# stm233/image-compression-for-machine

Hardware: AMD Instinct MI355X
Metric: images/sec (256x256) cnn-hyperprior (WACNN) training step (higher is better)
Workload: dtype f32; 1 GPU; cnn (WACNN N=192 M=320) train step, lambda=0.0067 MSE, batch 16/GPU synthetic 256x256, Adam lr 1e-4 + aux Adam, clip 1.0; global_batch=16, parallelism=dp1

## Files before the change

image-compression-for-machine_amd/csrc/conv_common.h:

```cpp
#pragma once
#include <type_traits>
#include "icm_common.h"

namespace icm {

#define ICM_MAX_TAPS 32
#define ICM_MAX_GROUPS 12

struct ConvPtrs {
  const float* x;
  const float* wp;
  const float* bias;
  float* y;
  const float* res;
  const float* aux;
  const float* aux2;
  float* y2;
};

struct ConvDesc {
  ConvPtrs g[ICM_MAX_GROUPS];
  long long y_bs, res_bs, aux_bs, aux2_bs, y2_bs;
  PatchGeom pg;
  int Cout, OHf, OWf;
// ... 81 lines not shown
template <int... Kinds>
struct EpiKinds {
  static constexpr bool has(int epi) { return ((epi == Kinds) || ...); }
  template <class F>
  static __device__ __forceinline__ void dispatch(int epi, F&& f) {
    static_assert(((Kinds == ICM_EPI_NONE) || ...), "ICM_EPI_NONE is the fallback of every kernel");
    const bool hit = ((Kinds != ICM_EPI_NONE && epi == Kinds ? (f(std::integral_constant<int, Kinds>{}), true) : false) || ...);
    if (!hit) f(std::integral_constant<int, ICM_EPI_NONE>{});
  }
};
using EpiAll = EpiKinds<ICM_EPI_NONE, ICM_EPI_RES, ICM_EPI_RES_GELU, ICM_EPI_GDN, ICM_EPI_IGDN, ICM_EPI_MUL_DGELU,
                        ICM_EPI_AXPY2, ICM_EPI_LRP, ICM_EPI_RES_MUL_DGELU>;
using EpiKs8 = EpiKinds<ICM_EPI_NONE, ICM_EPI_RES, ICM_EPI_RES_GELU, ICM_EPI_MUL_DGELU, ICM_EPI_LRP, ICM_EPI_RES_MUL_DGELU>;
using EpiWino = EpiKinds<ICM_EPI_NONE, ICM_EPI_RES, ICM_EPI_RES_GELU, ICM_EPI_MUL_DGELU, ICM_EPI_RES_MUL_DGELU, ICM_EPI_LRP>;

template <int EPI, int half>
__device__ __forceinline__ void store_half_e(const ConvDesc& d, const ConvPtrs& P, const f32x16 acc, int cot, int h,
                                             int n, int oy, int ox, bool pvalid) {
  const int plane = d.OHf * d.OWf;
  constexpr bool kRes = epi_reads_res(EPI), kAux = epi_reads_aux(EPI), kAux2 = epi_reads_aux2(EPI);
  float* yb = P.y + n * d.y_bs;
  const float* resb = kRes ? P.res + n * d.res_bs : nullptr;
  const float* auxb = kAux ? P.aux + n * d.aux_bs : nullptr;
  const float* aux2b = kAux2 ? P.aux2 + n * d.aux2_bs : nullptr;
  float* y2b = P.y2 ? P.y2 + n * d.y2_bs : nullptr;
  const bool has_bias = P.bias != nullptr;
  {
    int off[8];
    bool ok[8];
    float bv[8], rv[8], av[8];
#pragma unroll
    for (int q = 0; q < 8; ++q) {
      const int r = half * 8 + q;
      const int co = cot * 32 + (r & 3) + 8 * (r >> 2) + 4 * h;
      ok[q] = pvalid && co < d.Cout;
      off[q] = d.ps2 ? (co >> 2) * plane + (oy * 2 + ((co >> 1) & 1)) * d.OWf + ox * 2 + (co & 1)
                     : co * plane + oy * d.OWf + ox;
      bv[q] = (has_bias && ok[q]) ? P.bias[co] : 0.0f;
      if constexpr (kRes) rv[q] = ok[q] ? resb[off[q]] : 0.0f;
      if constexpr (kAux) av[q] = ok[q] ? auxb[off[q]] : 0.0f;
      if constexpr (kAux2) rv[q] = ok[q] ? aux2b[off[q]] : 0.0f;
    }
    float v[8];
#pragma unroll
    for (int q = 0; q < 8; ++q) {
      float side;
      v[q] = epi_apply<EPI>(acc[half * 8 + q] + bv[q], (kRes || kAux2) ? rv[q] : 0.0f, kAux ? av[q] : 0.0f, side);
      if constexpr (epi_writes_side(EPI))
        if (y2b && ok[q]) y2b[off[q]] = side;
    }
    if (d.accum) {
      float old[8];
#pragma unroll
      for (int q = 0; q < 8; ++q) old[q] = ok[q] ? yb[off[q]] : 0.0f;
#pragma unroll
      for (int q = 0; q < 8; ++q) v[q] += old[q];
    }
    if constexpr (epi_may_gelu(EPI)) {
      if (y2b) {
#pragma unroll
        for (int q = 0; q < 8; ++q) epi_materialise(v[q], yb, y2b, off[q], ok[q]);
      }
    }
#pragma unroll
    for (int q = 0; q < 8; ++q)
      if (ok[q]) yb[off[q]] = v[q];
  }
}
template <int EPI>
__device__ __forceinline__ void store_tile_e(const ConvDesc& d, const ConvPtrs& P, const f32x16 acc, int cot, int h,
                                             int n, int oy, int ox, bool pvalid) {
  store_half_e<EPI, 0>(d, P, acc, cot, h, n, oy, ox, pvalid);
  store_half_e<EPI, 1>(d, P, acc, cot, h, n, oy, ox, pvalid);
}

struct EpiRegs {
  int n;
  int off[8];
  bool ok[8];
  float bv[8], rv[8], av[8], old[8];
};

// ... 87 lines not shown
    epi_finish<EPI>(d, P, a8, R[i & 1]);
    __builtin_amdgcn_sched_barrier(0);
  }
}

template <int TCO, int TPX, bool PIPE2 = false>
__device__ __forceinline__ void epilogue_dispatch(const ConvDesc& d, const ConvPtrs& P, const f32x16 (&acc)[TCO][TPX],
                                                  int cot0, int h, const int (&pn)[TPX], const int (&poy)[TPX],
                                                  const int (&pox)[TPX], const bool (&pv)[TPX]) {
  EpiAll::dispatch(d.epi, [&](auto kind) {
    constexpr int EPI = decltype(kind)::value;
    epilogue_tiles<EPI, TCO, TPX, EPI == ICM_EPI_AXPY2 && PIPE2>(d, P, acc, cot0, h, pn, poy, pox, pv);
  });
}

int launch_conv_ks8(const ConvDesc& d, int tco, long long nblk, int ngroups, size_t lds_bytes, hipStream_t stream);

bool wino_supported(const icm_conv_args& a);
int plan_conv_wino(const icm_conv_args& a, int ngroups, WinoPlan& p);
int run_conv_wino(const icm_conv_args* arr, int ngroups, hipStream_t stream);
long long wino_transform_floats(const icm_conv_args& a);
int run_wino_transform(const icm_conv_args* arr, int ngroups, hipStream_t stream);

int plan_conv1x1(const icm_conv_args& a, int ngroups, int force_mode, ConvPlan& p);
int launch_conv1x1(ConvDesc& d, const icm_conv_args& a, const ConvPlan& p, int ngroups, hipStream_t stream);

}
```

image-compression-for-machine_amd/csrc/conv_igemm.hip:

```cpp
#include <cstdlib>
#include <vector>
#include "conv_common.h"

namespace icm {

template <int WCO, int WPX, int TCO, int TPX, int KS = 1>
__global__ __launch_bounds__(512, (TCO * TPX <= 3) ? 4 : 2) void conv_igemm_kernel(const ConvDesc d) {
  extern __shared__ __attribute__((aligned(16))) float smem[];
  static_assert(WCO * WPX * KS == 4, "4 MFMA waves per workgroup");
  constexpr int BCO_T = WCO * TCO;
  constexpr int TS = (TCO * TPX == 1) ? 3 : ((TCO * TPX == 2) ? 2 : 1);
  const int tid = threadIdx.x, lane = tid & 63, wave = tid >> 6;
  const bool loader = wave >= 4;
  const ConvPtrs P = d.g[blockIdx.y];
  const PatchGeom& pg = d.pg;

  int bid = xcd_block_id();
  const int cb = bid % d.ncb;
  int pt = bid / d.ncb;
  const int tx_i = pt % d.tiles_x;
  pt /= d.tiles_x;
  const int ty_i = pt % d.tiles_y;
  const int tn_i = pt / d.tiles_y;
  const int ox0 = tx_i << d.lgTW, oy0 = ty_i << d.lgTH, n0 = tn_i << d.lgTI;
// ... 460 lines not shown
  static const long long ks8_min = env_ll("ICM_CONV_KS8_MINWG", 160);
  if (!(ks8_forced() || (ks8_on && !cfg_forced())) || S_in != 1 || s.ntaps <= 1 || a.pro_act != ICM_ACT_NONE ||
      !EpiKs8::has(a.epi) || a.x_seg_len != 0)
    return 0;
  const int tco = g_force_cfg == ICM_CONV_CFG_KS8_32X128 ? 1 : (g_force_cfg == ICM_CONV_CFG_KS8_64X64 ? 2 : (s.ncot >= 2 ? 2 : 1));
  g = make_geometry(tco == 2 ? 64 : 128, s.OHv, s.OWv, a.N, S_in, cls.ey, cls.ex, s.nchunks8, s.ntaps, 4);
  int ckm = std::max(1, std::min(s.nchunks8, 64 / s.ntaps));
  while (ckm > 1 && (size_t)2 * ckm * 8 * g.CS * sizeof(float) > 96 * 1024) --ckm;
  g.ckm = ckm;
  g.lds_bytes = std::max((size_t)2 * ckm * 8 * g.CS * sizeof(float), (size_t)8 * 4 * 16 * 64 * sizeof(float));
  const long long blocks = cdiv(s.ncot, tco) * tile_count(g) * ngroups;
  const bool fits = g.lds_bytes <= 160 * 1024 && fits_plane_map(g) && linear_patch(g);
  return (fits && (ks8_forced() || (blocks <= ks8_max && blocks >= ks8_min && tco == 2))) ? tco : 0;
}

static int plan_class(const icm_conv_args& a, int ngroups, const ConvClass& cls, int S_in, int out_s, bool x_aligned16,
                      ConvPlan& p) {
  p = ConvPlan{};
  const ClassShape s = class_shape(a, cls, out_s);
  if (s.OHv <= 0 || s.OWv <= 0) return ICM_OK;
  if (s.ntaps > ICM_MAX_TAPS) return ICM_ERR_UNSUPPORTED;
  if (s.ntaps == 1 && S_in == 1 && out_s == 1 && cls.iy0 == 0 && cls.ix0 == 0 && a.x_seg_len == 0 && !cfg_forced()) {
    const int rc = plan_conv1x1(a, ngroups, g_force_1x1, p);
    if (rc >= 0) return rc;
  }
  p.row = search_staged(a, ngroups, cls, s, S_in, p.g);
  if (p.row < 0) return ICM_ERR_UNSUPPORTED;
  p.block = 512;
  Geometry kg;
  if (const int tco = plan_ks8(a, ngroups, cls, s, S_in, kg)) {
    p.family = kFamKs8;
    p.row = tco;
    p.g = kg;
    p.dma = 1;
  } else {
    const Geometry& g = p.g;
// ... 35 lines not shown
  d.OHf = d.ps2 ? a.OH * 2 : a.OH;
  d.OWf = d.ps2 ? a.OW * 2 : a.OW;
  d.OHv = s.OHv; d.OWv = s.OWv;
  d.out_sy = d.out_sx = out_s;
  d.out_oy = cls.cy; d.out_ox = cls.cx;
  d.iy0 = cls.iy0; d.ix0 = cls.ix0;
  d.ntaps = s.ntaps;
  d.lgTW = bg.lgTW; d.lgTH = bg.lgTH; d.lgTI = bg.lgTI;
  d.tiles_x = bg.tiles_x; d.tiles_y = bg.tiles_y; d.tiles_n = bg.tiles_n;
  d.nchunks8 = s.nchunks8; d.ckm = bg.ckm;
  for (int t = 0; t < s.ntaps; ++t) {
    const Tap& tp = cls.taps[t];
    const int col = (S_in == 2) ? ((tp.dx & 1) * bg.PWh + (tp.dx >> 1)) : tp.dx;
    d.tapoff[t] = tp.dy * bg.PWrow + col;
  }
  if (p.family == kFamKs8) return launch_conv_ks8(d, p.row, p.nblk, ngroups, bg.lds_bytes, stream);
  const KernelCfg& c = kCfgs[p.row];
  if (bg.lds_bytes > 64 * 1024 && !ensure_max_lds(reinterpret_cast<const void*>(c.fn))) return ICM_ERR_LAUNCH;
  hipLaunchKernelGGL(c.fn, dim3((unsigned)p.nblk, ngroups, 1), dim3(p.block), bg.lds_bytes, stream, d);
  ICM_CHECK_LAUNCH();
  return ICM_OK;
}

static int validate(const icm_conv_args& a) {
  if (!a.x || !a.wp || !a.y) return ICM_ERR_ARG;
  if (a.N <= 0 || a.Cin <= 0 || a.Cout <= 0 || a.H <= 0 || a.W <= 0 || a.OH <= 0 || a.OW <= 0) return ICM_ERR_ARG;
  if (a.KH <= 0 || a.KW <= 0 || a.KH * a.KW > ICM_MAX_TAPS) return ICM_ERR_UNSUPPORTED;
  if (a.stride != 1 && a.stride != 2) return ICM_ERR_UNSUPPORTED;
  if (!a.transposed) {
    if (a.OH != (a.H + 2 * a.pad - a.KH) / a.stride + 1 || a.OW != (a.W + 2 * a.pad - a.KW) / a.stride + 1)
      return ICM_ERR_ARG;
// ... 14 lines not shown
    if (rc) return rc;
  }
  const icm_conv_args& a = arr[0];
  for (int i = 1; i < ngroups; ++i) {
    const icm_conv_args& b = arr[i];
    if (b.N != a.N || b.Cin != a.Cin || b.H != a.H || b.W != a.W || b.Cout != a.Cout || b.OH != a.OH || b.OW != a.OW ||
        b.KH != a.KH || b.KW != a.KW || b.stride != a.stride || b.pad != a.pad || b.transposed != a.transposed ||
        b.pro_act != a.pro_act || b.epi != a.epi || b.accum != a.accum || b.pixel_shuffle != a.pixel_shuffle ||
        b.x_bs != a.x_bs || b.y_bs != a.y_bs || b.x_seg_len != a.x_seg_len || b.x_seg_gap != a.x_seg_gap || b.algo != a.algo ||
        (b.res && b.res_bs != a.res_bs) || (b.aux && b.aux_bs != a.aux_bs) || (b.aux2 && b.aux2_bs != a.aux2_bs) ||
        (b.y2 && b.y2_bs != a.y2_bs) || (b.res != nullptr) != (a.res != nullptr) || (b.aux != nullptr) != (a.aux != nullptr) ||
        (b.aux2 != nullptr) != (a.aux2 != nullptr) || (b.y2 != nullptr) != (a.y2 != nullptr) ||
        (b.bias != nullptr) != (a.bias != nullptr) || (b.xv != nullptr) != (a.xv != nullptr))
      return ICM_ERR_ARG;
  }
  return (a.algo == ICM_ALGO_WINOGRAD || a.algo == ICM_ALGO_DIRECT) ? ICM_OK : ICM_ERR_ARG;
}

static long long class_packed_floats(int Cin, int ntaps, int ncot) { return (long long)cdiv(Cin, 8) * ntaps * ncot * 256; }

static bool x_aligned16(const icm_conv_args* arr, int ngroups) {
  bool ok = true;
  for (int gi = 0; gi < ngroups; ++gi) ok = ok && (reinterpret_cast<uintptr_t>(arr[gi].x) & 15) == 0;
  return ok;
}

static int conv_run_grouped(const icm_conv_args* arr, int ngroups, hipStream_t stream) {
  if (int rc = check_group(arr, ngroups)) return rc;
  const icm_conv_args& a = arr[0];
  if (a.algo == ICM_ALGO_WINOGRAD) return run_conv_wino(arr, ngroups, stream);
  const int S_in = a.transposed ? 1 : a.stride, out_s = a.transposed ? a.stride : 1;
// ... 38 lines not shown
}
int icm_convT2d_dgrad(const icm_conv_args* a, void* stream) {
  if (!a || a->transposed) return ICM_ERR_ARG;
  return icm_conv_run(a, stream);
}
int icm_conv2d_dgrad(const icm_conv_args* a, void* stream) {
  if (!a || !a->transposed) return ICM_ERR_ARG;
  return icm_conv_run(a, stream);
}
int icm_convT2d_fwd(const icm_conv_args* a, void* stream) {
  if (!a || !a->transposed) return ICM_ERR_ARG;
  return icm_conv_run(a, stream);
}

int icm_conv_winograd_ok(const icm_conv_args* a) { return (a && icm::wino_supported(*a)) ? 1 : 0; }
int64_t icm_wino_transform_floats(const icm_conv_args* a) {
  return (a && icm::wino_supported(*a) && a->N > 0 && a->Cin > 0) ? (int64_t)icm::wino_transform_floats(*a) : -1;
}
int icm_wino_transform(const icm_conv_args* arr, int ngroups, void* stream) {
  if (!arr || ngroups < 1 || ngroups > ICM_MAX_GROUPS) return ICM_ERR_ARG;
  for (int i = 1; i < ngroups; ++i)
    if (arr[i].N != arr[0].N || arr[i].Cin != arr[0].Cin || arr[i].H != arr[0].H || arr[i].W != arr[0].W ||
        arr[i].x_bs != arr[0].x_bs || arr[i].pro_act != arr[0].pro_act || arr[i].x_seg_len != arr[0].x_seg_len ||
        arr[i].x_seg_gap != arr[0].x_seg_gap)
      return ICM_ERR_ARG;
  return icm::run_wino_transform(arr, ngroups, (hipStream_t)stream);
}

void icm_debug_force_conv_cfg(int idx) { icm::g_force_cfg = idx < 0 ? ICM_CONV_CFG_AUTO : idx; }
int icm_debug_forced_conv_cfg(void) { return icm::g_force_cfg; }
// ... 98 lines not shown
```

image-compression-for-machine_amd/csrc/conv_ks8.hip:

```cpp
#include <cstdlib>
#include "conv_common.h"

namespace icm {

template <int EPI>
__device__ __forceinline__ void ks8_store(const ConvDesc& d, const ConvPtrs& P, const f32x16 v, int cot, int hf, int h, int n,
                                          int oy, int ox, bool pvalid) {
  if (hf == 0) store_half_e<EPI, 0>(d, P, v, cot, h, n, oy, ox, pvalid);
  else store_half_e<EPI, 1>(d, P, v, cot, h, n, oy, ox, pvalid);
}

template <int TCO, int TPX>
__global__ __launch_bounds__(512, 2) void conv_ks8_kernel(const ConvDesc d) {
  extern __shared__ __attribute__((aligned(16))) float smem[];
  static_assert(TCO * TPX == 4, "four output tiles per workgroup: one half tile per wave in the epilogue");
  const int tid = threadIdx.x, lane = tid & 63;
  const int wave = __builtin_amdgcn_readfirstlane(tid >> 6);
  const ConvPtrs P = d.g[blockIdx.y];
  const PatchGeom& pg = d.pg;
  int bid = xcd_block_id();
  const int cb = bid % d.ncb;
  int pt = bid / d.ncb;
  const int tx_i = pt % d.tiles_x;
  pt /= d.tiles_x;
  const int ty_i = pt % d.tiles_y;
  const int tn_i = pt / d.tiles_y;
  const int ox0 = tx_i << d.lgTW, oy0 = ty_i << d.lgTH, n0 = tn_i << d.lgTI;
  const int iyb = oy0 + d.iy0, ixb = ox0 + d.ix0;
  const int bufsz = d.ckm * 8 * pg.CS;
  const int nchunks = (d.nchunks8 + d.ckm - 1) / d.ckm;
  const long long HWb = (long long)pg.H * pg.W * 4;
  const float* zero = icm_zero_page + lane;
  const int nj = (pg.TIPH * pg.PW + 63) >> 6;

  PlaneMap pm;
  plane_map_init(pm, pg, n0, iyb, ixb, lane);
  const char* xb = reinterpret_cast<const char*>(P.x);
  auto stage = [&](int chunk) {
    const int c0 = chunk * d.ckm * 8;
    const int nch = min(d.ckm, d.nchunks8 - chunk * d.ckm) * 8;
    float* dst = smem + (chunk & 1) * bufsz;
    for (int cl = wave; cl < nch; cl += 8) {
      const int c = c0 + cl;
      const char* base = xb + (long long)c * HWb;
      float* slab = dst + cl * pg.CS;
#pragma unroll
      for (int j = 0; j < ICM_MAXJ; ++j) {
        if (j < nj && pm.loff[j] >= 0) {
          const float* pp = (c < pg.C && pm.goff[j] >= 0) ? reinterpret_cast<const float*>(base + pm.goff[j]) : zero;
          __builtin_amdgcn_global_load_lds(pp, slab + 64 * j, 4, 0, 0);
        }
      }
    }
  };

  const int h = lane >> 5, l31 = lane & 31;
  const int TWm = (1 << d.lgTW) - 1, THm = (1 << d.lgTH) - 1;
  int boff[TPX];
#pragma unroll
// ... 65 lines not shown
            acc[a][tp] = __builtin_amdgcn_mfma_f32_32x32x2f32(aq[u][a][j], bv[j][tp], acc[a][tp], 0, 0, 0);
        aq[u][a] = *reinterpret_cast<const f32x4*>(sp + wl[a]);
      }
    }
  }
  while (chunk + 1 < nchunks) cross();
  asm volatile("s_waitcnt vmcnt(0)" ::: "memory");
  __syncthreads();

  float* red = smem;
#pragma unroll
  for (int a = 0; a < TCO; ++a)
#pragma unroll
    for (int tp = 0; tp < TPX; ++tp)
#pragma unroll
      for (int r = 0; r < 16; ++r) red[((wave * 4 + a * TPX + tp) * 16 + r) * 64 + lane] = acc[a][tp][r];
  __syncthreads();
  const int t = wave >> 1, hf = wave & 1;
  f32x16 v;
#pragma unroll
  for (int r = 0; r < 16; ++r) v[r] = 0.0f;
#pragma unroll
  for (int q = 0; q < 8; ++q) {
    float s = 0.0f;
#pragma unroll
    for (int k = 0; k < 8; ++k) s += red[((k * 4 + t) * 16 + hf * 8 + q) * 64 + lane];
    if (hf == 0) v[q] = s; else v[8 + q] = s;
  }
  const int a_t = t / TPX, tp_t = t % TPX;
  const int cot = cot0 + a_t;
  const int p = tp_t * 32 + l31;
  const int tx = p & TWm, ty = (p >> d.lgTW) & THm, ti = p >> (d.lgTW + d.lgTH);
  const int n = n0 + ti, oyv = oy0 + ty, oxv = ox0 + tx;
  const bool pvalid = (n < pg.N) && (oyv < d.OHv) && (oxv < d.OWv) && cot < d.ncot;
  const int oy = oyv * d.out_sy + d.out_oy, ox = oxv * d.out_sx + d.out_ox;
  EpiKs8::dispatch(d.epi, [&](auto kind) { ks8_store<decltype(kind)::value>(d, P, v, cot, hf, h, n, oy, ox, pvalid); });
}

int launch_conv_ks8(const ConvDesc& d, int tco, long long nblk, int ngroups, size_t lds_bytes, hipStream_t stream) {
  void (*fn)(const ConvDesc) = tco == 2 ? conv_ks8_kernel<2, 2> : conv_ks8_kernel<1, 4>;
  if (lds_bytes > 64 * 1024 && !ensure_max_lds(reinterpret_cast<const void*>(fn))) return ICM_ERR_LAUNCH;
  hipLaunchKernelGGL(fn, dim3((unsigned)nblk, ngroups, 1), dim3(512), lds_bytes, stream, d);
  ICM_CHECK_LAUNCH();
  return ICM_OK;
}

}
```

image-compression-for-machine_amd/icm_amd/_lib.py:

```python
from __future__ import annotations

import ctypes as C
import os

import torch

_HERE = os.path.dirname(os.path.abspath(__file__))
LIB_PATH = os.environ.get("ICM_LIB", os.path.join(os.path.dirname(_HERE), "lib", "libicm_hip.so"))

ACT_NONE, ACT_GELU, ACT_SQUARE = 0, 1, 2
CONV_CFG_AUTO, CONV_CFG_KS8_64X64, CONV_CFG_KS8_32X128 = -1, 100, 101
TILE_EDGE_LEFT, TILE_EDGE_RIGHT, TILE_EDGE_TOP, TILE_EDGE_BOTTOM = 1, 2, 4, 8
EPI_NONE, EPI_RES, EPI_RES_GELU, EPI_GDN, EPI_IGDN, EPI_MUL_DGELU, EPI_AXPY2, EPI_LRP, EPI_RES_MUL_DGELU = range(9)

_f = C.POINTER(C.c_float)
i64, i32, f32, vp = C.c_int64, C.c_int, C.c_float, C.c_void_p


class ConvArgs(C.Structure):
    _fields_ = [
        ("x", vp), ("x_bs", i64), ("N", i32), ("Cin", i32), ("H", i32), ("W", i32),
        ("wp", vp), ("bias", vp),
        ("y", vp), ("y_bs", i64), ("Cout", i32), ("OH", i32), ("OW", i32),
        ("KH", i32), ("KW", i32), ("stride", i32), ("pad", i32),
        ("transposed", i32), ("pro_act", i32), ("epi", i32),
        ("res", vp), ("res_bs", i64), ("aux", vp), ("aux_bs", i64), ("aux2", vp), ("aux2_bs", i64),
# ... 26 lines not shown
    _fields_ = [("matrix", vp * 5), ("bias", vp * 5), ("factor", vp * 4), ("dmedian", vp)]


class IcmError(RuntimeError):
    pass


_lib = None

SYMBOLS = [
    "icm_strerror", "icm_version", "icm_conv_run", "icm_conv_run_grouped", "icm_conv2d_fwd", "icm_conv2d_dgrad",
    "icm_convT2d_fwd", "icm_convT2d_dgrad", "icm_packed_weight_floats", "icm_pack_weights", "icm_pack_weights_batch",
    "icm_wgrad_workspace_floats", "icm_wgrad_workspace_floats_grouped", "icm_conv_wgrad", "icm_conv_wgrad_grouped", "icm_channel_sum", "icm_nonneg_fwd", "icm_nonneg_bwd",
    "icm_gdn_bwd_pre", "icm_gelu_fwd", "icm_gate_fwd", "icm_gate_bwd", "icm_add_grad", "icm_ste_round_offset",
    "icm_lrp_bwd", "icm_pixel_unshuffle2", "icm_layernorm_fwd", "icm_layernorm_bwd", "icm_space_to_depth2",
    "icm_residual_scale", "icm_im2col", "icm_col2im", "icm_copy_strided", "icm_permute_flip", "icm_gather_vectors", "icm_conv_winograd_ok", "icm_wino_transform_floats", "icm_wino_transform", "icm_winattn_fwd", "icm_winattn_bwd",
    "icm_eb_likelihood_fwd", "icm_eb_likelihood_bwd", "icm_eb_aux_loss", "icm_gc_likelihood_ste_fwd",
    "icm_gc_likelihood_ste_bwd", "icm_rd_loss_fwd", "icm_rd_loss_bwd", "icm_grad_sqnorm", "icm_adam_step", "icm_adam_step_hyper", "icm_fill",
    "icm_winattn_bwd_workspace_floats", "icm_debug_force_conv_cfg", "icm_debug_forced_conv_cfg", "icm_debug_force_conv1x1",
    "icm_debug_force_wgrad_cfg", "icm_debug_wgrad_plan", "icm_debug_conv_plan",
    "icm_debug_force_winattn_valu", "icm_debug_winattn_route",
    "icm_zigzag_order", "icm_zigzag_splits", "icm_zigzag_reverse",
    "icm_pmf_to_quantized_cdf", "icm_rans_encode_with_indexes", "icm_rans_decode_with_indexes",
    "icm_rans_decoder_create", "icm_rans_decoder_decode", "icm_rans_decoder_destroy",
    "icm_rans_lanes_waves", "icm_rans_lanes_encode", "icm_rans_lanes_decoder_create",
    "icm_rans_lanes_decoder_decode_run", "icm_rans_lanes_decoder_finish", "icm_rans_lanes_decoder_destroy",
    "icm_rans_lanes_encode_gpu_workspace", "icm_rans_lanes_encode_gpu", "icm_rans_lanes_decoder_gpu_create",
    "icm_rans_lanes_decoder_gpu_decode_run", "icm_rans_lanes_decoder_gpu_finish", "icm_rans_lanes_decoder_gpu_destroy",
    "icm_debug_lanes_search",
    "icm_eb_table_bounds", "icm_eb_pmf_table", "icm_gc_table_centers", "icm_gc_pmf_table", "icm_gc_build_indexes",
    "icm_quantize", "icm_dequantize", "icm_clamp", "icm_pad2d",
# ... 11 lines not shown
    if _lib is None:
        if not os.path.exists(LIB_PATH):
            raise IcmError(
                f"{LIB_PATH} not found: build it with image-compression-for-machine_amd/build.sh "
                "(hipcc --offload-arch=gfx950). There is no CPU fallback.")
        L = C.CDLL(LIB_PATH)
        L.icm_strerror.restype = C.c_char_p
        L.icm_packed_weight_floats.restype = i64
        L.icm_wgrad_workspace_floats.restype = i64
        L.icm_wgrad_workspace_floats_grouped.restype = i64
        L.icm_packed_weight_floats.argtypes = [i32, i32, i32, i32]
        L.icm_pack_weights.argtypes = [vp, vp, i32, i32, i32, i32, i32, i32, i32, i32, i32, f32, f32, vp]
        L.icm_pack_weights_batch.argtypes = [C.POINTER(PackJob), i32, vp]
        L.icm_conv_run.argtypes = [C.POINTER(ConvArgs), vp]
        L.icm_conv_winograd_ok.argtypes = [C.POINTER(ConvArgs)]
        L.icm_wino_transform_floats.argtypes = [C.POINTER(ConvArgs)]
        L.icm_wino_transform_floats.restype = i64
        L.icm_wino_transform.argtypes = [C.POINTER(ConvArgs), i32, vp]
        L.icm_conv_run_grouped.argtypes = [C.POINTER(ConvArgs), i32, vp]
        for n in ("icm_conv2d_fwd", "icm_conv2d_dgrad", "icm_convT2d_fwd", "icm_convT2d_dgrad"):
            getattr(L, n).argtypes = [C.POINTER(ConvArgs), vp]
        L.icm_wgrad_workspace_floats.argtypes = [C.POINTER(WgradArgs)]
        L.icm_wgrad_workspace_floats_grouped.argtypes = [C.POINTER(WgradArgs), i32]
        L.icm_conv_wgrad.argtypes = [C.POINTER(WgradArgs), vp]
        L.icm_conv_wgrad_grouped.argtypes = [C.POINTER(WgradArgs), i32, vp]
        L.icm_channel_sum.argtypes = [vp, i64, i32, i32, i32, vp, i32, vp, i64, vp]
        L.icm_gather_vectors.argtypes = [C.POINTER(vp), i32, i32, vp, vp]
        L.icm_nonneg_fwd.argtypes = [vp, vp, i64, f32, f32, vp]
        L.icm_nonneg_bwd.argtypes = [vp, vp, vp, i64, f32, i32, vp]
        L.icm_gdn_bwd_pre.argtypes = [vp, vp, vp, vp, vp, i64, i32, vp]
# ... 138 lines not shown
```

image-compression-for-machine_amd/icm_amd/engine.py:

```python
from __future__ import annotations

import ctypes as C
import os as _os
from typing import Callable, Dict, List, Optional, Sequence, Tuple

import torch

from . import _lib as L
from ._lib import (ACT_GELU, ACT_NONE, ACT_SQUARE, EPI_AXPY2, EPI_GDN, EPI_IGDN, EPI_LRP, EPI_MUL_DGELU, EPI_NONE,
                   EPI_RES, EPI_RES_GELU, EPI_RES_MUL_DGELU, bs, check, ptr)
from .bitstream import step_of, step_table

PEDESTAL = 2.0 ** -36
_SKIP_WGRAD = _os.environ.get("ICM_DEBUG_SKIP_WGRAD", "0") == "1"
PAIR_GATE_BRANCHES = _os.environ.get("ICM_PAIR_GATE_BRANCHES", "1") == "1"


MAX_GROUP = 12


USE_WINO = _os.environ.get("ICM_WINO", "1") != "0"
_WINO_MIN_CIN = int(_os.environ.get("ICM_WINO_MIN_CIN", "96"))
_WINO_MIN_WORK = float(_os.environ.get("ICM_WINO_MIN_WORK", "2.0e8"))
_WINO_WG_BATCH = float(_os.environ.get("ICM_WINO_WG_BATCH", "4"))
USE_WINO_WGRAD = _os.environ.get("ICM_WINO_WGRAD", "1") != "0"
THIN_OUT = _os.environ.get("ICM_THIN_OUT", "1") != "0"
EVAL_INPLACE_ACT = _os.environ.get("ICM_EVAL_INPLACE_ACT", "1") != "0"
WINO_PRE = _os.environ.get("ICM_WINO_PRE", "1") != "0"
_WINO_WG_MAX_PIXELS = int(_os.environ.get("ICM_WINO_WG_MAX_PIXELS", "100000"))


_WINO_WG_MIN_C = int(_os.environ.get("ICM_WINO_WG_MIN_C", "64"))


def wino_ok(KH, KW, stride, pad, Cin, ps=0, conv_transposed=False, work: float = 1e30, min_c=None) -> bool:
    return (USE_WINO and KH == 3 and KW == 3 and stride == 1 and pad == 1 and not ps and not conv_transposed and
            Cin >= (_WINO_MIN_CIN if min_c is None else min_c) and work >= _WINO_MIN_WORK and
            L.lib().icm_debug_forced_conv_cfg() == L.CONV_CFG_AUTO)


_weight_gen = [0]


def bump_weight_generation():
    _weight_gen[0] += 1


PROFILE: Optional[list] = None


def _prof_begin(stream=None):
    if PROFILE is None:
        return None
# ... 278 lines not shown
        a.accum, a.pixel_shuffle, a.algo = accum, ps, algo
        if biases is not None:
            a.bias = ptr(biases[i])
        if ress is not None:
            a.res, a.res_bs = ptr(ress[i]), bs(ress[i])
        if auxs is not None:
            a.aux, a.aux_bs = ptr(auxs[i]), bs(auxs[i])
        if aux2s is not None:
            a.aux2, a.aux2_bs = ptr(aux2s[i]), bs(aux2s[i])
        if y2s is not None:
            a.y2, a.y2_bs = ptr(y2s[i]), bs(y2s[i])
        if seg is not None:
            a.x_seg_len, a.x_seg_gap = seg
    if n > 1 and len({(m.x_bs, m.y_bs, m.res_bs, m.aux_bs, m.aux2_bs, m.y2_bs) for m in arr}) > 1:
        raise ValueError("grouped conv: members must share strides")
    if algo and WINO_PRE:
        _wino_pretransform(tape, arr, xs)
    if single:
        check(L.lib().icm_conv_run(C.byref(arr[0]), tape.st), "conv_run")
    else:
        check(L.lib().icm_conv_run_grouped(arr, n, tape.st), "conv_run_grouped")
    if e0 is not None:
        N, _, H, W = xs[0].shape
        px = H * W if transposed else OH * OW
        _prof_end(e0, _conv_label(tag + ("/wino" if algo else ""), transposed, KH, stride, Cin, Cout, H, W, N, n),
                  2.0 * n * N * Cin * Cout * KH * KW * px)


def conv_launch_grouped(tape, xs, wps, biases, ys, **kw):
    _conv_launch(tape, False, xs, wps, biases, ys, **kw)


def conv_launch(tape, x, wp, bias, y, *, res=None, aux=None, aux2=None, y2=None, **kw):
    one = lambda t: None if t is None else (t,)
    _conv_launch(tape, True, (x,), (wp,), one(bias), (y,), ress=one(res), auxs=one(aux), aux2s=one(aux2), y2s=one(y2),
                 **kw)


def _wgrad_args(a, gs, gb, dw, geom, accum, dbias, accum_bias, dw_ld=0, algo=0):
    Ca, Cb, KH, KW, stride, pad, act_s, act_b, N, OH, OW, H, W, gs_bs, gb_bs = geom
# ... 875 lines not shown
```

include/icm_hip.h:

```cpp
#ifndef ICM_HIP_H
#define ICM_HIP_H
#include <stdint.h>

#ifdef __cplusplus
extern "C" {
#endif

#define ICM_OK 0
#define ICM_ERR_ARG 1
#define ICM_ERR_LAUNCH 2
#define ICM_ERR_UNSUPPORTED 3

#define ICM_ACT_NONE 0
#define ICM_ACT_GELU 1
#define ICM_ACT_SQUARE 2

#define ICM_EPI_NONE 0
#define ICM_EPI_RES 1
#define ICM_EPI_RES_GELU 2
#define ICM_EPI_GDN 3
#define ICM_EPI_IGDN 4
#define ICM_EPI_MUL_DGELU 5
#define ICM_EPI_AXPY2 6
#define ICM_EPI_LRP 7
// ... 11 lines not shown
  int transposed;
  int pro_act;
  int epi;
  const float* res; int64_t res_bs;
  const float* aux; int64_t aux_bs;
  const float* aux2; int64_t aux2_bs;
  float* y2; int64_t y2_bs;
  int accum;
  int pixel_shuffle;
  int x_seg_len, x_seg_gap;
  int algo;
  float* xv;
} icm_conv_args;
#define ICM_ALGO_DIRECT 0
#define ICM_ALGO_WINOGRAD 1
int icm_conv_winograd_ok(const icm_conv_args* a);
int64_t icm_wino_transform_floats(const icm_conv_args* a);
int icm_wino_transform(const icm_conv_args* arr, int ngroups, void* stream);

int icm_conv_run(const icm_conv_args* a, void* stream);
int icm_conv_run_grouped(const icm_conv_args* a, int ngroups, void* stream);
int icm_conv2d_fwd(const icm_conv_args* a, void* stream);
int icm_conv2d_dgrad(const icm_conv_args* a, void* stream);
int icm_convT2d_fwd(const icm_conv_args* a, void* stream);
int icm_convT2d_dgrad(const icm_conv_args* a, void* stream);

int64_t icm_packed_weight_floats(int Cout, int Cin, int KH, int KW);
int icm_pack_weights(const float* w, float* wp, int Cout, int Cin, int KH, int KW, int src_out_major,
                     int transposed, int stride, int pad, int nonneg, float bound, float pedestal,
                     void* stream);

// ... 199 lines not shown
#define ICM_TILE_EDGE_LEFT 1
#define ICM_TILE_EDGE_RIGHT 2
#define ICM_TILE_EDGE_TOP 4
#define ICM_TILE_EDGE_BOTTOM 8
int icm_image_tile_blend(const float* src, int PH, int PW, int top, int left, int h, int w,
                         float* canvas, int H, int W, int y0, int x0,
                         const float* ramp, int m, int edges, void* stream);

typedef struct { int64_t offset; int32_t H, W, y0, x0; } icm_crop_desc;
int icm_image_batch_u8_to_f32(const uint8_t* arena, const icm_crop_desc* desc, int B, float* dst ,
                              int CH, int CW, void* stream);

#define ICM_CONV_CFG_AUTO (-1)
#define ICM_CONV_CFG_KS8_64X64 100
#define ICM_CONV_CFG_KS8_32X128 101
void icm_debug_force_conv_cfg(int idx);
int icm_debug_forced_conv_cfg(void);
void icm_debug_force_conv1x1(int mode);
int icm_debug_conv_plan(const icm_conv_args* a, int ngroups, int cls, int64_t out[16]);
void icm_debug_force_wgrad_cfg(int variant, int xcd_order);
int icm_debug_wgrad_plan(const icm_wgrad_args* a, int n, int32_t out[8]);
void icm_debug_force_winattn_valu(int on);
int icm_debug_winattn_route(int N, int C, int H, int W, int heads, int ws, int shift, int backward);

#ifdef __cplusplus
}
#endif
#endif
```

Measured before the change: 386.7 images/s.

## Add split-K conv path with smaller tile shapes for low-occupancy layers

Adds an ICM_ALGO_KSPLIT path that routes small-tile-count convolutions to the 8-wave split-K kernel. The kernel is generalized to 1, 2 or 4 output tiles per workgroup, and a planner picks the shape that best fills one round of workgroups. The Python engine enables the path by default for layers within tile, step and Cout thresholds. The aim is better GPU occupancy on small-spatial layers whose tile count underfills the device, at the cost of an LDS reduction across waves and heuristic thresholds that may misroute some layers.

```diff
diff --git a/image-compression-for-machine_amd/csrc/conv_common.h b/image-compression-for-machine_amd/csrc/conv_common.h
--- a/image-compression-for-machine_amd/csrc/conv_common.h
+++ b/image-compression-for-machine_amd/csrc/conv_common.h
@@ -119,9 +119,9 @@
 using EpiKs8 = EpiKinds<ICM_EPI_NONE, ICM_EPI_RES, ICM_EPI_RES_GELU, ICM_EPI_MUL_DGELU, ICM_EPI_LRP, ICM_EPI_RES_MUL_DGELU>;
 using EpiWino = EpiKinds<ICM_EPI_NONE, ICM_EPI_RES, ICM_EPI_RES_GELU, ICM_EPI_MUL_DGELU, ICM_EPI_RES_MUL_DGELU, ICM_EPI_LRP>;
 
-template <int EPI, int half>
-__device__ __forceinline__ void store_half_e(const ConvDesc& d, const ConvPtrs& P, const f32x16 acc, int cot, int h,
-                                             int n, int oy, int ox, bool pvalid) {
+template <int EPI, int NR>
+__device__ __forceinline__ void store_rows_e(const ConvDesc& d, const ConvPtrs& P, const float (&a8)[NR], int r0, int cot,
+                                             int h, int n, int oy, int ox, bool pvalid) {
   const int plane = d.OHf * d.OWf;
   constexpr bool kRes = epi_reads_res(EPI), kAux = epi_reads_aux(EPI), kAux2 = epi_reads_aux2(EPI);
   float* yb = P.y + n * d.y_bs;
@@ -131,12 +131,12 @@
   float* y2b = P.y2 ? P.y2 + n * d.y2_bs : nullptr;
   const bool has_bias = P.bias != nullptr;
   {
-    int off[8];
-    bool ok[8];
-    float bv[8], rv[8], av[8];
-#pragma unroll
-    for (int q = 0; q < 8; ++q) {
-      const int r = half * 8 + q;
+    int off[NR];
+    bool ok[NR];
+    float bv[NR], rv[NR], av[NR];
+#pragma unroll
+    for (int q = 0; q < NR; ++q) {
+      const int r = r0 + q;
       const int co = cot * 32 + (r & 3) + 8 * (r >> 2) + 4 * h;
       ok[q] = pvalid && co < d.Cout;
       off[q] = d.ps2 ? (co >> 2) * plane + (oy * 2 + ((co >> 1) & 1)) * d.OWf + ox * 2 + (co & 1)
@@ -146,31 +146,39 @@
       if constexpr (kAux) av[q] = ok[q] ? auxb[off[q]] : 0.0f;
       if constexpr (kAux2) rv[q] = ok[q] ? aux2b[off[q]] : 0.0f;
     }
-    float v[8];
-#pragma unroll
-    for (int q = 0; q < 8; ++q) {
+    float v[NR];
+#pragma unroll
+    for (int q = 0; q < NR; ++q) {
       float side;
-      v[q] = epi_apply<EPI>(acc[half * 8 + q] + bv[q], (kRes || kAux2) ? rv[q] : 0.0f, kAux ? av[q] : 0.0f, side);
+      v[q] = epi_apply<EPI>(a8[q] + bv[q], (kRes || kAux2) ? rv[q] : 0.0f, kAux ? av[q] : 0.0f, side);
       if constexpr (epi_writes_side(EPI))
         if (y2b && ok[q]) y2b[off[q]] = side;
     }
     if (d.accum) {
-      float old[8];
-#pragma unroll
-      for (int q = 0; q < 8; ++q) old[q] = ok[q] ? yb[off[q]] : 0.0f;
-#pragma unroll
-      for (int q = 0; q < 8; ++q) v[q] += old[q];
+      float old[NR];
+#pragma unroll
+      for (int q = 0; q < NR; ++q) old[q] = ok[q] ? yb[off[q]] : 0.0f;
+#pragma unroll
+      for (int q = 0; q < NR; ++q) v[q] += old[q];
     }
     if constexpr (epi_may_gelu(EPI)) {
       if (y2b) {
 #pragma unroll
-        for (int q = 0; q < 8; ++q) epi_materialise(v[q], yb, y2b, off[q], ok[q]);
+        for (int q = 0; q < NR; ++q) epi_materialise(v[q], yb, y2b, off[q], ok[q]);
       }
     }
 #pragma unroll
-    for (int q = 0; q < 8; ++q)
+    for (int q = 0; q < NR; ++q)
       if (ok[q]) yb[off[q]] = v[q];
   }
+}
+template <int EPI, int half>
+__device__ __forceinline__ void store_half_e(const ConvDesc& d, const ConvPtrs& P, const f32x16 acc, int cot, int h,
+                                             int n, int oy, int ox, bool pvalid) {
+  float a8[8];
+#pragma unroll
+  for (int q = 0; q < 8; ++q) a8[q] = acc[half * 8 + q];
+  store_rows_e<EPI, 8>(d, P, a8, half * 8, cot, h, n, oy, ox, pvalid);
 }
 template <int EPI>
 __device__ __forceinline__ void store_tile_e(const ConvDesc& d, const ConvPtrs& P, const f32x16 acc, int cot, int h,
@@ -288,7 +296,8 @@
   });
 }
 
-int launch_conv_ks8(const ConvDesc& d, int tco, long long nblk, int ngroups, size_t lds_bytes, hipStream_t stream);
+constexpr size_t ks8_fold_bytes(int tiles) { return (size_t)8 * tiles * 16 * 64 * sizeof(float); }
+int launch_conv_ks8(const ConvDesc& d, int tco, int tpx, long long nblk, int ngroups, size_t lds_bytes, hipStream_t stream);
 
 bool wino_supported(const icm_conv_args& a);
 int plan_conv_wino(const icm_conv_args& a, int ngroups, WinoPlan& p);
diff --git a/image-compression-for-machine_amd/csrc/conv_igemm.hip b/image-compression-for-machine_amd/csrc/conv_igemm.hip
--- a/image-compression-for-machine_amd/csrc/conv_igemm.hip
+++ b/image-compression-for-machine_amd/csrc/conv_igemm.hip
@@ -498,12 +498,53 @@
   return (fits && (ks8_forced() || (blocks <= ks8_max && blocks >= ks8_min && tco == 2))) ? tco : 0;
 }
 
+static const int kKsShapes[5][2] = {{2, 2}, {1, 4}, {2, 1}, {1, 2}, {1, 1}};
+static int ks_forced_shape() {
+  return (g_force_cfg >= ICM_CONV_CFG_KS8_64X64 && g_force_cfg <= ICM_CONV_CFG_KS8_32X32) ? g_force_cfg - ICM_CONV_CFG_KS8_64X64 : -1;
+}
+static int ks_occupancy(size_t lds_bytes) { return (int)std::max<size_t>(1, std::min<size_t>(2, 160 * 1024 / lds_bytes)); }
+static int plan_ksplit(const icm_conv_args& a, int ngroups, const ConvClass& cls, const ClassShape& s, int S_in, ConvPlan& p) {
+  if (S_in != 1 || a.pro_act != ICM_ACT_NONE || !EpiKs8::has(a.epi) || s.ntaps > 64)
+    return ICM_ERR_UNSUPPORTED;
+  const int forced = ks_forced_shape();
+  long long best_cost = -1;
+  for (int i = 0; i < 5; ++i) {
+    if (forced >= 0 ? i != forced : kKsShapes[i][0] > s.ncot) continue;
+    const int tco = kKsShapes[i][0], tpx = kKsShapes[i][1], T = tco * tpx;
+    Geometry g = make_geometry(32 * tpx, s.OHv, s.OWv, a.N, S_in, cls.ey, cls.ex, s.nchunks8, s.ntaps, T);
+    const size_t stage_max = T == 4 ? 96 * 1024 : 80 * 1024;
+    int ckm = std::max(1, std::min(s.nchunks8, 64 / s.ntaps));
+    while (ckm > 1 && (size_t)2 * ckm * 8 * g.CS * sizeof(float) > stage_max) --ckm;
+    g.ckm = ckm;
+    g.lds_bytes = std::max((size_t)2 * ckm * 8 * g.CS * sizeof(float), ks8_fold_bytes(T));
+    if (g.lds_bytes > 160 * 1024 || !fits_plane_map(g) || !linear_patch(g)) continue;
+    const long long blocks = cdiv(s.ncot, tco) * tile_count(g) * ngroups;
+    const long long round = 256LL * ks_occupancy(g.lds_bytes);
+    const long long rounds = (blocks + round - 1) / round;
+    const long long cost = ((blocks + 255) / 256) * T + rounds + (rounds > 1 ? 1000000 : 0);
+    if (best_cost < 0 || cost < best_cost) {
+      best_cost = cost;
+      p.row = tco;
+      p.g = g;
+    }
+  }
+  if (best_cost < 0) return ICM_ERR_UNSUPPORTED;
+  p.family = kFamKs8;
+  p.block = 512;
+  p.dma = 1;
+  p.ncb = cdiv(s.ncot, p.row);
+  p.nblk = p.ncb * tile_count(p.g);
+  if (p.nblk <= 0 || p.nblk > 0x7fffffffLL) return ICM_ERR_ARG;
+  return ICM_OK;
+}
+
 static int plan_class(const icm_conv_args& a, int ngroups, const ConvClass& cls, int S_in, int out_s, bool x_aligned16,
                       ConvPlan& p) {
   p = ConvPlan{};
   const ClassShape s = class_shape(a, cls, out_s);
   if (s.OHv <= 0 || s.OWv <= 0) return ICM_OK;
   if (s.ntaps > ICM_MAX_TAPS) return ICM_ERR_UNSUPPORTED;
+  if (a.algo == ICM_ALGO_KSPLIT) return plan_ksplit(a, ngroups, cls, s, S_in, p);
   if (s.ntaps == 1 && S_in == 1 && out_s == 1 && cls.iy0 == 0 && cls.ix0 == 0 && a.x_seg_len == 0 && !cfg_forced()) {
     const int rc = plan_conv1x1(a, ngroups, g_force_1x1, p);
     if (rc >= 0) return rc;
@@ -569,7 +610,8 @@
     const int col = (S_in == 2) ? ((tp.dx & 1) * bg.PWh + (tp.dx >> 1)) : tp.dx;
     d.tapoff[t] = tp.dy * bg.PWrow + col;
   }
-  if (p.family == kFamKs8) return launch_conv_ks8(d, p.row, p.nblk, ngroups, bg.lds_bytes, stream);
+  if (p.family == kFamKs8)
+    return launch_conv_ks8(d, p.row, (1 << (bg.lgTW + bg.lgTH + bg.lgTI)) / 32, p.nblk, ngroups, bg.lds_bytes, stream);
   const KernelCfg& c = kCfgs[p.row];
   if (bg.lds_bytes > 64 * 1024 && !ensure_max_lds(reinterpret_cast<const void*>(c.fn))) return ICM_ERR_LAUNCH;
   hipLaunchKernelGGL(c.fn, dim3((unsigned)p.nblk, ngroups, 1), dim3(p.block), bg.lds_bytes, stream, d);
@@ -614,7 +656,7 @@
         (b.bias != nullptr) != (a.bias != nullptr) || (b.xv != nullptr) != (a.xv != nullptr))
       return ICM_ERR_ARG;
   }
-  return (a.algo == ICM_ALGO_WINOGRAD || a.algo == ICM_ALGO_DIRECT) ? ICM_OK : ICM_ERR_ARG;
+  return (a.algo == ICM_ALGO_WINOGRAD || a.algo == ICM_ALGO_DIRECT || a.algo == ICM_ALGO_KSPLIT) ? ICM_OK : ICM_ERR_ARG;
 }
 
 static long long class_packed_floats(int Cin, int ntaps, int ncot) { return (long long)cdiv(Cin, 8) * ntaps * ncot * 256; }
@@ -683,6 +725,21 @@
 }
 
 int icm_conv_winograd_ok(const icm_conv_args* a) { return (a && icm::wino_supported(*a)) ? 1 : 0; }
+int icm_conv_ksplit_ok(const icm_conv_args* a, int ngroups) {
+  using namespace icm;
+  if (!a || ngroups < 1 || ngroups > ICM_MAX_GROUPS) return 0;
+  icm_conv_args q = *a;
+  q.x = q.wp = q.res = q.aux = q.aux2 = reinterpret_cast<const float*>(&q);
+  q.y = reinterpret_cast<float*>(&q);
+  q.algo = ICM_ALGO_KSPLIT;
+  if (validate(q) != ICM_OK) return 0;
+  const int S_in = q.transposed ? 1 : q.stride, out_s = q.transposed ? q.stride : 1;
+  for (const ConvClass& cls : build_classes(q.KH, q.KW, q.stride, q.pad, q.transposed)) {
+    ConvPlan p;
+    if (plan_class(q, ngroups, cls, S_in, out_s, false, p) != ICM_OK) return 0;
+  }
+  return 1;
+}
 int64_t icm_wino_transform_floats(const icm_conv_args* a) {
   return (a && icm::wino_supported(*a) && a->N > 0 && a->Cin > 0) ? (int64_t)icm::wino_transform_floats(*a) : -1;
 }
diff --git a/image-compression-for-machine_amd/csrc/conv_ks8.hip b/image-compression-for-machine_amd/csrc/conv_ks8.hip
--- a/image-compression-for-machine_amd/csrc/conv_ks8.hip
+++ b/image-compression-for-machine_amd/csrc/conv_ks8.hip
@@ -3,17 +3,13 @@
 
 namespace icm {
 
-template <int EPI>
-__device__ __forceinline__ void ks8_store(const ConvDesc& d, const ConvPtrs& P, const f32x16 v, int cot, int hf, int h, int n,
-                                          int oy, int ox, bool pvalid) {
-  if (hf == 0) store_half_e<EPI, 0>(d, P, v, cot, h, n, oy, ox, pvalid);
-  else store_half_e<EPI, 1>(d, P, v, cot, h, n, oy, ox, pvalid);
-}
-
 template <int TCO, int TPX>
 __global__ __launch_bounds__(512, 2) void conv_ks8_kernel(const ConvDesc d) {
   extern __shared__ __attribute__((aligned(16))) float smem[];
-  static_assert(TCO * TPX == 4, "four output tiles per workgroup: one half tile per wave in the epilogue");
+  constexpr int T = TCO * TPX;
+  constexpr int WPT = 8 / T;
+  constexpr int NR = 2 * T;
+  static_assert(T == 1 || T == 2 || T == 4, "the eight waves share the 16 rows of every tile evenly");
   const int tid = threadIdx.x, lane = tid & 63;
   const int wave = __builtin_amdgcn_readfirstlane(tid >> 6);
   const ConvPtrs P = d.g[blockIdx.y];
@@ -42,7 +38,7 @@
     float* dst = smem + (chunk & 1) * bufsz;
     for (int cl = wave; cl < nch; cl += 8) {
       const int c = c0 + cl;
-      const char* base = xb + (long long)c * HWb;
+      const char* base = xb + (long long)phys_ch(pg, c) * HWb;
       float* slab = dst + cl * pg.CS;
 #pragma unroll
       for (int j = 0; j < ICM_MAXJ; ++j) {
@@ -138,18 +134,16 @@
 #pragma unroll
     for (int tp = 0; tp < TPX; ++tp)
 #pragma unroll
-      for (int r = 0; r < 16; ++r) red[((wave * 4 + a * TPX + tp) * 16 + r) * 64 + lane] = acc[a][tp][r];
+      for (int r = 0; r < 16; ++r) red[((wave * T + a * TPX + tp) * 16 + r) * 64 + lane] = acc[a][tp][r];
   __syncthreads();
-  const int t = wave >> 1, hf = wave & 1;
-  f32x16 v;
+  const int t = wave / WPT, r0 = (wave % WPT) * NR;
+  float v[NR];
 #pragma unroll
-  for (int r = 0; r < 16; ++r) v[r] = 0.0f;
-#pragma unroll
-  for (int q = 0; q < 8; ++q) {
+  for (int q = 0; q < NR; ++q) {
     float s = 0.0f;
 #pragma unroll
-    for (int k = 0; k < 8; ++k) s += red[((k * 4 + t) * 16 + hf * 8 + q) * 64 + lane];
-    if (hf == 0) v[q] = s; else v[8 + q] = s;
+    for (int k = 0; k < 8; ++k) s += red[((k * T + t) * 16 + r0 + q) * 64 + lane];
+    v[q] = s;
   }
   const int a_t = t / TPX, tp_t = t % TPX;
   const int cot = cot0 + a_t;
@@ -158,11 +152,18 @@
   const int n = n0 + ti, oyv = oy0 + ty, oxv = ox0 + tx;
   const bool pvalid = (n < pg.N) && (oyv < d.OHv) && (oxv < d.OWv) && cot < d.ncot;
   const int oy = oyv * d.out_sy + d.out_oy, ox = oxv * d.out_sx + d.out_ox;
-  EpiKs8::dispatch(d.epi, [&](auto kind) { ks8_store<decltype(kind)::value>(d, P, v, cot, hf, h, n, oy, ox, pvalid); });
+  EpiKs8::dispatch(d.epi, [&](auto kind) { store_rows_e<decltype(kind)::value, NR>(d, P, v, r0, cot, h, n, oy, ox, pvalid); });
 }
 
-int launch_conv_ks8(const ConvDesc& d, int tco, long long nblk, int ngroups, size_t lds_bytes, hipStream_t stream) {
-  void (*fn)(const ConvDesc) = tco == 2 ? conv_ks8_kernel<2, 2> : conv_ks8_kernel<1, 4>;
+int launch_conv_ks8(const ConvDesc& d, int tco, int tpx, long long nblk, int ngroups, size_t lds_bytes, hipStream_t stream) {
+  void (*fn)(const ConvDesc) = nullptr;
+  if (tco == 2 && tpx == 2) fn = conv_ks8_kernel<2, 2>;
+  else if (tco == 1 && tpx == 4) fn = conv_ks8_kernel<1, 4>;
+  else if (tco == 2 && tpx == 1) fn = conv_ks8_kernel<2, 1>;
+  else if (tco == 1 && tpx == 2) fn = conv_ks8_kernel<1, 2>;
+  else if (tco == 1 && tpx == 1) fn = conv_ks8_kernel<1, 1>;
+  else return ICM_ERR_UNSUPPORTED;
+  if (lds_bytes < ks8_fold_bytes(tco * tpx)) return ICM_ERR_ARG;
   if (lds_bytes > 64 * 1024 && !ensure_max_lds(reinterpret_cast<const void*>(fn))) return ICM_ERR_LAUNCH;
   hipLaunchKernelGGL(fn, dim3((unsigned)nblk, ngroups, 1), dim3(512), lds_bytes, stream, d);
   ICM_CHECK_LAUNCH();
diff --git a/image-compression-for-machine_amd/icm_amd/_lib.py b/image-compression-for-machine_amd/icm_amd/_lib.py
--- a/image-compression-for-machine_amd/icm_amd/_lib.py
+++ b/image-compression-for-machine_amd/icm_amd/_lib.py
@@ -10,6 +10,8 @@
 
 ACT_NONE, ACT_GELU, ACT_SQUARE = 0, 1, 2
 CONV_CFG_AUTO, CONV_CFG_KS8_64X64, CONV_CFG_KS8_32X128 = -1, 100, 101
+CONV_CFG_KS8_64X32, CONV_CFG_KS8_32X64, CONV_CFG_KS8_32X32 = 102, 103, 104
+ALGO_DIRECT, ALGO_WINOGRAD, ALGO_KSPLIT = 0, 1, 3
 TILE_EDGE_LEFT, TILE_EDGE_RIGHT, TILE_EDGE_TOP, TILE_EDGE_BOTTOM = 1, 2, 4, 8
 EPI_NONE, EPI_RES, EPI_RES_GELU, EPI_GDN, EPI_IGDN, EPI_MUL_DGELU, EPI_AXPY2, EPI_LRP, EPI_RES_MUL_DGELU = range(9)
 
@@ -66,7 +68,7 @@
     "icm_wgrad_workspace_floats", "icm_wgrad_workspace_floats_grouped", "icm_conv_wgrad", "icm_conv_wgrad_grouped", "icm_channel_sum", "icm_nonneg_fwd", "icm_nonneg_bwd",
     "icm_gdn_bwd_pre", "icm_gelu_fwd", "icm_gate_fwd", "icm_gate_bwd", "icm_add_grad", "icm_ste_round_offset",
     "icm_lrp_bwd", "icm_pixel_unshuffle2", "icm_layernorm_fwd", "icm_layernorm_bwd", "icm_space_to_depth2",
-    "icm_residual_scale", "icm_im2col", "icm_col2im", "icm_copy_strided", "icm_permute_flip", "icm_gather_vectors", "icm_conv_winograd_ok", "icm_wino_transform_floats", "icm_wino_transform", "icm_winattn_fwd", "icm_winattn_bwd",
+    "icm_residual_scale", "icm_im2col", "icm_col2im", "icm_copy_strided", "icm_permute_flip", "icm_gather_vectors", "icm_conv_winograd_ok", "icm_conv_ksplit_ok", "icm_wino_transform_floats", "icm_wino_transform", "icm_winattn_fwd", "icm_winattn_bwd",
     "icm_eb_likelihood_fwd", "icm_eb_likelihood_bwd", "icm_eb_aux_loss", "icm_gc_likelihood_ste_fwd",
     "icm_gc_likelihood_ste_bwd", "icm_rd_loss_fwd", "icm_rd_loss_bwd", "icm_grad_sqnorm", "icm_adam_step", "icm_adam_step_hyper", "icm_fill",
     "icm_winattn_bwd_workspace_floats", "icm_debug_force_conv_cfg", "icm_debug_forced_conv_cfg", "icm_debug_force_conv1x1",
@@ -108,6 +110,7 @@
         L.icm_pack_weights_batch.argtypes = [C.POINTER(PackJob), i32, vp]
         L.icm_conv_run.argtypes = [C.POINTER(ConvArgs), vp]
         L.icm_conv_winograd_ok.argtypes = [C.POINTER(ConvArgs)]
+        L.icm_conv_ksplit_ok.argtypes = [C.POINTER(ConvArgs), i32]
         L.icm_wino_transform_floats.argtypes = [C.POINTER(ConvArgs)]
         L.icm_wino_transform_floats.restype = i64
         L.icm_wino_transform.argtypes = [C.POINTER(ConvArgs), i32, vp]
diff --git a/image-compression-for-machine_amd/icm_amd/engine.py b/image-compression-for-machine_amd/icm_amd/engine.py
--- a/image-compression-for-machine_amd/icm_amd/engine.py
+++ b/image-compression-for-machine_amd/icm_amd/engine.py
@@ -37,6 +37,34 @@
     return (USE_WINO and KH == 3 and KW == 3 and stride == 1 and pad == 1 and not ps and not conv_transposed and
             Cin >= (_WINO_MIN_CIN if min_c is None else min_c) and work >= _WINO_MIN_WORK and
             L.lib().icm_debug_forced_conv_cfg() == L.CONV_CFG_AUTO)
+
+
+USE_KSPLIT = _os.environ.get("ICM_KSPLIT", "1") != "0"
+_KSPLIT_MAX_TILES = int(_os.environ.get("ICM_KSPLIT_MAX_TILES", "2560"))
+_KSPLIT_MIN_STEPS = int(_os.environ.get("ICM_KSPLIT_MIN_STEPS", "36"))
+_KSPLIT_MAX_STEPS = int(_os.environ.get("ICM_KSPLIT_MAX_STEPS", "200"))
+_KSPLIT_MIN_MAP = int(_os.environ.get("ICM_KSPLIT_MIN_MAP", "256"))
+_KSPLIT_MAX_COUT = int(_os.environ.get("ICM_KSPLIT_MAX_COUT", "192"))
+_KSPLIT_1X1 = _os.environ.get("ICM_KSPLIT_1X1", "0") != "0"
+_KSPLIT_EPIS = (EPI_NONE, EPI_RES, EPI_RES_GELU, EPI_MUL_DGELU, EPI_LRP, EPI_RES_MUL_DGELU)
+_ksplit_seen = {}
+
+
+def ksplit_ok(a, n, algo=0) -> bool:
+    if not USE_KSPLIT or algo or a.pro_act != ACT_NONE or a.epi not in _KSPLIT_EPIS:
+        return False
+    key = (a.N, a.Cin, a.H, a.W, a.Cout, a.OH, a.OW, a.KH, a.KW, a.stride, a.pad, a.transposed, a.epi, a.pixel_shuffle, n,
+           a.x_seg_len, a.x_seg_gap)
+    ok = _ksplit_seen.get(key)
+    if ok is None:
+        s2 = a.stride * a.stride if a.transposed else 1
+        tiles = -(-a.Cout // 32) * -(-a.N * a.OH * a.OW // (32 * s2)) * n
+        steps = -(-a.Cin // 8) * max(1, a.KH * a.KW // s2)
+        ok = _ksplit_seen[key] = bool(tiles <= _KSPLIT_MAX_TILES and _KSPLIT_MIN_STEPS <= steps <= _KSPLIT_MAX_STEPS and
+                                      (a.KH * a.KW > 1 or _KSPLIT_1X1) and a.OH * a.OW >= _KSPLIT_MIN_MAP * s2 and
+                                      a.Cout <= _KSPLIT_MAX_COUT and (a.transposed or a.stride == 1) and
+                                      L.lib().icm_conv_ksplit_ok(C.byref(a), n))
+    return ok and L.lib().icm_debug_forced_conv_cfg() == L.CONV_CFG_AUTO
 
 
 _weight_gen = [0]
@@ -345,7 +373,11 @@
             a.x_seg_len, a.x_seg_gap = seg
     if n > 1 and len({(m.x_bs, m.y_bs, m.res_bs, m.aux_bs, m.aux2_bs, m.y2_bs) for m in arr}) > 1:
         raise ValueError("grouped conv: members must share strides")
-    if algo and WINO_PRE:
+    ks = ksplit_ok(arr[0], n, algo)
+    if ks:
+        for a in arr:
+            a.algo = L.ALGO_KSPLIT
+    elif algo and WINO_PRE:
         _wino_pretransform(tape, arr, xs)
     if single:
         check(L.lib().icm_conv_run(C.byref(arr[0]), tape.st), "conv_run")
@@ -354,7 +386,7 @@
     if e0 is not None:
         N, _, H, W = xs[0].shape
         px = H * W if transposed else OH * OW
-        _prof_end(e0, _conv_label(tag + ("/wino" if algo else ""), transposed, KH, stride, Cin, Cout, H, W, N, n),
+        _prof_end(e0, _conv_label(tag + ("/wino" if algo else "/ks" if ks else ""), transposed, KH, stride, Cin, Cout, H, W, N, n),
                   2.0 * n * N * Cin * Cout * KH * KW * px)
 
 
diff --git a/include/icm_hip.h b/include/icm_hip.h
--- a/include/icm_hip.h
+++ b/include/icm_hip.h
@@ -49,7 +49,9 @@
 } icm_conv_args;
 #define ICM_ALGO_DIRECT 0
 #define ICM_ALGO_WINOGRAD 1
+#define ICM_ALGO_KSPLIT 3
 int icm_conv_winograd_ok(const icm_conv_args* a);
+int icm_conv_ksplit_ok(const icm_conv_args* a, int ngroups);
 int64_t icm_wino_transform_floats(const icm_conv_args* a);
 int icm_wino_transform(const icm_conv_args* arr, int ngroups, void* stream);
 
@@ -279,6 +281,9 @@
 #define ICM_CONV_CFG_AUTO (-1)
 #define ICM_CONV_CFG_KS8_64X64 100
 #define ICM_CONV_CFG_KS8_32X128 101
+#define ICM_CONV_CFG_KS8_64X32 102
+#define ICM_CONV_CFG_KS8_32X64 103
+#define ICM_CONV_CFG_KS8_32X32 104
 void icm_debug_force_conv_cfg(int idx);
 int icm_debug_forced_conv_cfg(void);
 void icm_debug_force_conv1x1(int mode);
```

Result: slower. 381.6 images/s (-1.3%).
